# yanielc/medical-vision-textural-bias

Hardware: AMD Instinct MI355X
Metric: BraTS 4ch 240^3 vols/sec filtered+train-step @1/2/4/8 GPU; filter HBM GB/s (higher is better)
Workload: dtype f32

## Files before the change

include/texbias.h:

```cpp
#ifndef TEXBIAS_H
#define TEXBIAS_H

#include <stddef.h>
#include <stdint.h>

#ifdef __cplusplus
extern "C" {
#endif

#define TB_VERSION 1

#define TB_OK 0
#define TB_ERR_INVALID_ARG 1
#define TB_ERR_UNSUPPORTED_SIZE 2
#define TB_ERR_HIP 3
#define TB_ERR_WORKSPACE 4

#define TB_OP_NONE 0
#define TB_OP_DISK 1
#define TB_OP_GIBBS 2
#define TB_OP_LAYER 3
#define TB_OP_WRAP 4
#define TB_OP_SPIKE 5
#define TB_OP_ZF 6
// ... 37 lines not shown

int tb_salt_pepper_f32(const float* x, float* y, int8_t* cls, const float* u_in, uint64_t seed, uint64_t offset,
                       const float* thr, const uint32_t* minmax, int B, int64_t rows, int len, int64_t ld,
                       int64_t sb, void* stream);

int tb_minmax_f32(const float* x, uint32_t* minmax, int B, int64_t rows, int len, int64_t ld, int64_t sb,
                  void* stream);

float tb_key_to_float(uint32_t key);

int tb_disk_mask_f32(float* mask, int64_t outer, int n0, int n1, int n2, int int_r, int64_t r2i, float r2f,
                     int inside_off, void* stream);

int tb_kspace_logabs_sum_f32(const tb_plan* plan, const float* x, const int64_t* xs, void* ws, size_t ws_bytes,
                             int B, int C, const tb_sample_ops* ops, double* out, void* stream);

int tb_conv3d_wgrad_f32(const float* G, const float* X, float* dW, int N, int M, int Cc, int Do, int Ho, int Wo, int Di,
                        int Hi, int Wi, int stride, int pad, void* stream);

int64_t tb_conv3d_wgrad_ws_bytes(int N, int M, int Cc, int Do, int Ho, int Wo, int Di, int Hi, int Wi, int stride,
                                 int pad);
int tb_conv3d_wgrad_ws_f32(const float* G, const float* X, float* dW, int N, int M, int Cc, int Do, int Ho, int Wo,
                           int Di, int Hi, int Wi, int stride, int pad, void* ws, size_t ws_bytes, void* stream);

int tb_conv3d_wgrad_config(int N, int M, int Cc, int Do, int Ho, int Wo, int Di, int Hi, int Wi, int stride, int pad,
                           int64_t* cfg);

int tb_dice_sums_f32(const float* x, const float* t, double* sums, int64_t NC, int64_t S, int sigmoid, int squared,
                     void* stream);
size_t tb_dice_sums_ws_bytes(int64_t NC, int64_t S);
int tb_dice_sums_ws_f32(const float* x, const float* t, double* sums, int64_t NC, int64_t S, int sigmoid, int squared,
                        void* ws, size_t ws_bytes, void* stream);
int tb_dice_metric_sums_f32(const float* x, const float* t, double* sums, int64_t NC, int64_t S, void* stream);
int tb_dice_sums_bwd_f32(const float* x, const float* t, const float* g, float* dx, int64_t NC, int64_t S, int sigmoid,
                         int squared, void* stream);
int tb_dice_loss_f32(const double* sums, float* loss, int64_t NC, int64_t C, int batch, int reduction, float smooth_nr,
                     float smooth_dr, void* stream);
int tb_dice_loss_bwd_f32(const double* sums, const float* gloss, float* gsums, int64_t NC, int64_t C, int batch,
                         int reduction, float smooth_nr, float smooth_dr, void* stream);

int tb_channel_sum_f32(const float* x, float* out, int64_t N, int64_t C, int64_t S, void* stream);
size_t tb_channel_sum_ws_bytes(int64_t N, int64_t C, int64_t S);
int tb_channel_sum_ws_f32(const float* x, float* out, int64_t N, int64_t C, int64_t S, void* ws, size_t ws_bytes,
                          void* stream);

int tb_conv3d_small_f32(const float* x, const float* w, const float* b, float* y, int N, int Cin, int Cout, int D,
// ... 111 lines not shown
```

medical-vision-textural-bias_amd/csrc/conv_wgrad.hip:

```cpp
#include <hip/hip_runtime.h>

#include <cstdlib>

#include "num_cu.h"
#include "texbias.h"

namespace {

typedef float f32x4 __attribute__((ext_vector_type(4)));

constexpr int NT = 256;
constexpr int LDS_FLOATS = 78 * 1024 / 4;
constexpr int kSlack = 16;

struct WgArgs {
  const float* G;
  const float* X;
  float* dW;
  int M, Cc, Do, Ho, Wo, Di, Hi, Wi;
  int YB, YR, Wo4, XP, PG, PC, ncc, ctiles, nyb, xcols;
  int64_t nchunks;
};

typedef __attribute__((address_space(1))) const void* gptr_t;
// ... 390 lines not shown
  }
  __syncthreads();
  if (wave < 2) {
#pragma unroll
    for (int j = 0; j < 27; ++j)
#pragma unroll
      for (int rr = 0; rr < 4; ++rr) red[((j * 2 + wave) * 4 + rr) * 64 + lane] = acc[j][rr];
  }
  __syncthreads();
  float* pt = a.part ? a.part + ((int64_t)blockIdx.y * gridDim.x + blockIdx.x) * (16 * 16 * 27) : nullptr;
  for (int e = tid; e < 27 * 4 * 64; e += NT) {
    const int ln = e & 63, rr = (e >> 6) & 3, j = e >> 8;
    const int m = (ln >> 4) * 4 + rr, c = ln & 15;
    const float v = red[((j * 2 + 0) * 4 + rr) * 64 + ln] + red[((j * 2 + 1) * 4 + rr) * 64 + ln];
    if (pt) {
      pt[(m * 16 + c) * 27 + j] = v;
    } else if (m < mv && c < cv) {
      atomicAdd(&a.dW[((int64_t)(m0 + m) * a.Cc + (c0 + c)) * 27 + j], v);
    }
  }
}

__global__ __launch_bounds__(1024) void k_wgrad_reduce(const float* __restrict__ part, float* __restrict__ dW, int nblk,
                                                       int TM, int TC, int ctiles, int M, int Cc) {
  __shared__ float red[16][64];
  const int tid = (int)threadIdx.x, el = tid & 63, bg = tid >> 6;
  const int TE = TM * TC * 27, tile = (int)blockIdx.y;
  const int e = (int)blockIdx.x * 64 + el;
  const float* src = part + (int64_t)tile * nblk * TE + (e < TE ? e : 0);
  float s0 = 0.f, s1 = 0.f, s2 = 0.f, s3 = 0.f;
  int b = bg;
  for (; b + 48 < nblk; b += 64) {
    s0 += src[(int64_t)b * TE];
    s1 += src[(int64_t)(b + 16) * TE];
    s2 += src[(int64_t)(b + 32) * TE];
    s3 += src[(int64_t)(b + 48) * TE];
  }
  for (; b < nblk; b += 16) s0 += src[(int64_t)b * TE];
  red[bg][el] = (s0 + s1) + (s2 + s3);
  __syncthreads();
  if (bg == 0 && e < TE) {
    float v = 0.f;
#pragma unroll
    for (int g = 0; g < 16; ++g) v += red[g][el];
    const int mt = tile / ctiles, ct = tile - mt * ctiles;
    const int m = e / (TC * 27), r = e - m * (TC * 27), c = r / 27, j = r - c * 27;
    if (mt * TM + m < M && ct * TC + c < Cc) dW[((int64_t)(mt * TM + m) * Cc + ct * TC + c) * 27 + j] = v;
  }
}
// ... 333 lines not shown
    for (int j = 0; j < 9; ++j)
#pragma unroll
      for (int rr = 0; rr < 4; ++rr) red[(((t * 9 + j) * NW + wave) * 4 + rr) * 64 + lane] = acc[t][j][rr];
  __syncthreads();
  float* pt = a.part ? a.part + ((int64_t)blockIdx.y * gridDim.x + blockIdx.x) * (16 * MT * Cc * 27) : nullptr;
  for (int e = tid; e < MT * 9 * 4 * 64; e += NT) {
    const int ln = e & 63, rr = (e >> 6) & 3, tj = e >> 8, t = tj / 9, j = tj - 9 * t;
    const int m = 16 * t + (ln >> 4) * 4 + rr, col = ln & 15;
    if ((!pt && m >= mv) || col >= 3 * Cc) continue;
    float v = 0.f;
#pragma unroll
    for (int w = 0; w < NW; ++w) v += red[((tj * NW + w) * 4 + rr) * 64 + ln];
    const int c = col / 3, tx = col - 3 * c;
    if (pt) pt[(m * Cc + c) * 27 + j * 3 + tx] = v;
    else atomicAdd(&a.dW[((int64_t)(m0 + m) * Cc + c) * 27 + j * 3 + tx], v);
  }
}

struct Zf1Args {
  const float* G;
  const float* X;
  float* dW;
  float* part;
  int N, M, Cc, D, H, W;
  int YB, nyb, ZS, zlen;
  int GR, GM, GS;
  int XR, XC, XS;
};

template <int YB, int WV>
__global__ __launch_bounds__(256) void k_conv3d_wgrad_zf1(Zf1Args a) {
  extern __shared__ __attribute__((aligned(16))) float smem[];
  const int tid = (int)threadIdx.x, lane = tid & 63;
  const int wave = __builtin_amdgcn_readfirstlane(tid >> 6);
  const int W = a.W, H = a.H, D = a.D, M = a.M, Cc = a.Cc;
  float* gsl = smem;
  float* xsl = smem + 4 * a.GS;
  int b = (int)blockIdx.x;
  const int zs = b % a.ZS;
  b /= a.ZS;
  const int yb = b % a.nyb, n = b / a.nyb;
  const int y0 = yb * YB;
  const int z0 = zs * a.zlen, z1 = min(D, z0 + a.zlen);
  for (int i = tid; i < 4 * a.GS + 2 * a.XS; i += 256) smem[i] = 0.f;
  const int64_t plane = (int64_t)H * W, plane4 = plane / 4;
  const float* Gb = a.G + (int64_t)n * M * D * plane;
  const float* Xb = a.X + (int64_t)n * Cc * D * plane;
  const int W4v = W >> 2;
  constexpr int NXL = (5 * YB * WV + 255) / 256, NGL = (3 * (YB + 2) * WV + 255) / 256;
  int xg[NXL], xl[NXL], gg[NGL], gl[NGL];
#pragma unroll
  for (int j = 0; j < NXL; ++j) {
    const int i = tid + 256 * j;
    const int q = i % W4v, t = i / W4v, yy = t % YB, c = t / YB;
    const bool ok = c < Cc && y0 + yy < H;
    xg[j] = ok ? (int)(((int64_t)c * D) * plane4 + ((y0 + yy) * W + 4 * q) / 4) : -1;
    xl[j] = c * a.XC + yy * a.XR + 4 + 4 * q;
  }
#pragma unroll
  for (int j = 0; j < NGL; ++j) {
    const int i = tid + 256 * j;
    const int q = i % W4v, t = i / W4v, r = t % (YB + 2), m = t / (YB + 2);
    const int y = y0 - 1 + r;
    const bool ok = m < M && y >= 0 && y < H;
    gg[j] = ok ? (int)(((int64_t)m * D) * plane4 + (y * W + 4 * q) / 4) : -1;
    gl[j] = m * a.GM + r * a.GR + 4 * q;
  }
  constexpr int ZP = 3;
  float4 rx[ZP][NXL], rg[ZP][NGL];
  auto load_x = [&](int zi, float4 (&r)[NXL]) {
    const float4* src = reinterpret_cast<const float4*>(Xb) + (int64_t)(zi < D ? zi : D - 1) * plane4;
#pragma unroll
    for (int j = 0; j < NXL; ++j) {
      const float4 v = src[xg[j] < 0 ? 0 : xg[j]];
      r[j] = xg[j] < 0 ? make_float4(0.f, 0.f, 0.f, 0.f) : v;
    }
  };
  auto store_x = [&](int slot, const float4 (&r)[NXL]) {
#pragma unroll
    for (int j = 0; j < NXL; ++j)
      if (xg[j] >= 0) *reinterpret_cast<float4*>(xsl + slot * a.XS + xl[j]) = r[j];
  };
  auto load_g = [&](int pz, float4 (&r)[NGL]) {
    const bool in = pz >= 0 && pz < D;
    const float4* src = reinterpret_cast<const float4*>(Gb) + (int64_t)(in ? pz : 0) * plane4;
#pragma unroll
    for (int j = 0; j < NGL; ++j) {
      const float4 v = src[gg[j] < 0 ? 0 : gg[j]];
      r[j] = (in && gg[j] >= 0) ? v : make_float4(0.f, 0.f, 0.f, 0.f);
    }
  };
  auto store_g = [&](int slot, const float4 (&r)[NGL], int) {
#pragma unroll
    for (int j = 0; j < NGL; ++j)
      if (gg[j] >= 0) *reinterpret_cast<float4*>(gsl + slot * a.GS + gl[j]) = r[j];
  };
  __syncthreads();
  load_g(z0 - 1, rg[0]);
  store_g((z0 + 3) & 3, rg[0], z0 - 1);
  load_g(z0, rg[0]);
  store_g(z0 & 3, rg[0], z0);
#pragma unroll
  for (int p = 0; p < ZP; ++p) {
    load_x(z0 + p, rx[p]);
    load_g(z0 + p + 1, rg[p]);
  }
  const int li = lane & 15, lk = lane >> 4;
  int atz[2], aoff[2];
  bool aok[2];
#pragma unroll
  for (int t = 0; t < 2; ++t) {
    const int r = 16 * t + li, m = r / 9, tz = (r / 3) % 3, ty = r % 3;
    aok[t] = m < M;
    atz[t] = tz;
    aoff[t] = aok[t] ? m * a.GM + (2 - ty) * a.GR + lk : 0;
  }
  const int bc = li / 3, btx = li - 3 * bc;
  const bool bok = bc < Cc;
  const int boff = bok ? bc * a.XC + 3 + btx + lk : 0;
  const int kpr = W >> 2, np = 4 / YB, yy = wave % YB, part = wave / YB;
  const int kb = (kpr * part) / np, ke = (kpr * (part + 1)) / np;
  f32x4 acc[2][2];
#pragma unroll
  for (int t = 0; t < 2; ++t) acc[0][t] = acc[1][t] = f32x4{0.f, 0.f, 0.f, 0.f};
  auto step = [&](int zi, float4 (&rxp)[NXL], float4 (&rgp)[NGL]) {
    store_x(zi & 1, rxp);
    store_g((zi + 1) & 3, rgp, zi + 1);
    __syncthreads();
    if (zi + ZP < z1) {
      load_x(zi + ZP, rxp);
      load_g(zi + ZP + 1, rgp);
    }
    const float* ga0 = gsl + ((zi + 1 - atz[0]) & 3) * a.GS + aoff[0] + yy * a.GR;
    const float* ga1 = gsl + ((zi + 1 - atz[1]) & 3) * a.GS + aoff[1] + yy * a.GR;
    const float* xb = xsl + (zi & 1) * a.XS + boff + yy * a.XR;
    auto ld = [&](int k, float& v0, float& v1, float& u) {
      const int px = 4 * (k < ke ? k : ke - 1);
      v0 = aok[0] ? ga0[px] : 0.f;
      v1 = aok[1] ? ga1[px] : 0.f;
      u = bok ? xb[px] : 0.f;
    };
    if (kb < ke) {
      float p0, p1, pu, q0, q1, qu;
      ld(kb, p0, p1, pu);
      int k = kb;
      for (; k + 1 < ke; k += 2) {
        ld(k + 1, q0, q1, qu);
        acc[0][0] = __builtin_amdgcn_mfma_f32_16x16x4f32(p0, pu, acc[0][0], 0, 0, 0);
        acc[0][1] = __builtin_amdgcn_mfma_f32_16x16x4f32(p1, pu, acc[0][1], 0, 0, 0);
        ld(k + 2, p0, p1, pu);
        acc[1][0] = __builtin_amdgcn_mfma_f32_16x16x4f32(q0, qu, acc[1][0], 0, 0, 0);
        acc[1][1] = __builtin_amdgcn_mfma_f32_16x16x4f32(q1, qu, acc[1][1], 0, 0, 0);
      }
      if (k < ke) {
        acc[0][0] = __builtin_amdgcn_mfma_f32_16x16x4f32(p0, pu, acc[0][0], 0, 0, 0);
        acc[0][1] = __builtin_amdgcn_mfma_f32_16x16x4f32(p1, pu, acc[0][1], 0, 0, 0);
      }
    }
  };
  for (int zi = z0; zi < z1; zi += ZP) {
    step(zi, rx[0], rg[0]);
    if (zi + 1 < z1) step(zi + 1, rx[1], rg[1]);
    if (zi + 2 < z1) step(zi + 2, rx[2], rg[2]);
  }
  __syncthreads();
  float* red = smem;
#pragma unroll
  for (int t = 0; t < 2; ++t)
#pragma unroll
    for (int rr = 0; rr < 4; ++rr) red[((t * 4 + wave) * 4 + rr) * 64 + lane] = acc[0][t][rr] + acc[1][t][rr];
  __syncthreads();
  float* pt = a.part ? a.part + (int64_t)blockIdx.x * (M * Cc * 27) : nullptr;
  for (int e = tid; e < 2 * 4 * 64; e += 256) {
    const int ln = e & 63, rr = (e >> 6) & 3, t = e >> 8;
    const int r = 16 * t + 4 * (ln >> 4) + rr, col = ln & 15;
    const int m = r / 9, c = col / 3;
    if (m >= M || c >= Cc) continue;
    const int tz = (r / 3) % 3, ty = r % 3, tx = col - 3 * c;
    const float v = red[((t * 4 + 0) * 4 + rr) * 64 + ln] + red[((t * 4 + 1) * 4 + rr) * 64 + ln] +
                    red[((t * 4 + 2) * 4 + rr) * 64 + ln] + red[((t * 4 + 3) * 4 + rr) * 64 + ln];
    if (pt) pt[(m * Cc + c) * 27 + tz * 9 + ty * 3 + tx] = v;
    else atomicAdd(&a.dW[((int64_t)m * Cc + c) * 27 + tz * 9 + ty * 3 + tx], v);
  }
}

int pad_mod32(int v, int rem) {
  while ((v & 31) != rem) ++v;
  return v;
}

template <int S, int TX, int SEG>
int launch(const WgArgs& a, int blocks_y, size_t lds, hipStream_t st) {
  static const hipError_t attr = hipFuncSetAttribute(reinterpret_cast<const void*>(&k_conv3d_wgrad<S, TX, SEG>),
                                                     hipFuncAttributeMaxDynamicSharedMemorySize, 163840);
  if (attr != hipSuccess) return TB_ERR_HIP;
  constexpr int target = 512;
  int64_t gx = (target + blocks_y - 1) / blocks_y;
  if (gx > a.nchunks) gx = a.nchunks;
  if (gx < 1) gx = 1;
  hipLaunchKernelGGL((k_conv3d_wgrad<S, TX, SEG>), dim3((unsigned)gx, (unsigned)blocks_y), dim3(NT), lds, st, a);
  return hipGetLastError() == hipSuccess ? TB_OK : TB_ERR_HIP;
}

template <int S, int TX>
int launch_seg(const WgArgs& a, int seg, int by, size_t lds, hipStream_t st) {
  switch (seg) {
// ... 251 lines not shown
template <int YB, int MT>
int launch_zf2_t(const Zf2Args& a, size_t lds, dim3 grid, hipStream_t st) {
  auto kern = a.Wo <= 40 ? k_conv3d_wgrad_zf2<YB, MT, 10, 8> : k_conv3d_wgrad_zf2<YB, MT, 20, 8>;
  const hipError_t attr = hipFuncSetAttribute(reinterpret_cast<const void*>(kern),
                                              hipFuncAttributeMaxDynamicSharedMemorySize, 163840);
  if (attr != hipSuccess) return TB_ERR_HIP;
  hipLaunchKernelGGL(kern, grid, dim3(512), lds, st, a);
  return hipGetLastError() == hipSuccess ? TB_OK : TB_ERR_HIP;
}
int launch_zf2(const Zf2Args& a, int MT, size_t lds, dim3 grid, hipStream_t st) {
  if (MT == 1) return a.YB == 4 ? launch_zf2_t<4, 1>(a, lds, grid, st) : a.YB == 2 ? launch_zf2_t<2, 1>(a, lds, grid, st) : launch_zf2_t<1, 1>(a, lds, grid, st);
  return a.YB == 4 ? launch_zf2_t<4, 2>(a, lds, grid, st) : a.YB == 2 ? launch_zf2_t<2, 2>(a, lds, grid, st) : launch_zf2_t<1, 2>(a, lds, grid, st);
}

bool use_zf1(int M, int Cc, int stride, int Do, int Ho, int Wo, int Di, int Hi, int Wi, const void* G, const void* X) {
  constexpr bool on = true;
  return on && stride == 1 && M <= 3 && Cc <= 5 && Do == Di && Ho == Hi && Wo == Wi && Wo % 4 == 0 && Wo <= 256 &&
         (reinterpret_cast<uintptr_t>(G) & 15) == 0 && (reinterpret_cast<uintptr_t>(X) & 15) == 0;
}

int zf1_setup(Zf1Args& a, size_t& lds, dim3& grid, int N, int M, int Cc, int D, int H, int W, int ncu) {
  a.N = N; a.M = M; a.Cc = Cc; a.D = D; a.H = H; a.W = W;
  constexpr int yb_env = 0;
  a.GR = pad_mod32(W, 4);
  a.XR = pad_mod32(W + 8, 4);
  a.YB = 0;
  for (int yb : {2, 4, 1}) {
    if (yb_env && yb != yb_env) continue;
    const int gm = pad_mod32((yb + 2) * a.GR, 12), gs = pad_mod32(M * gm, 20);
    const int xc = pad_mod32(yb * a.XR, 8), xs = pad_mod32(Cc * xc, 16);
    const size_t bytes = (size_t)4 * (4 * gs + 2 * xs);
    if (bytes <= 81920) {
      a.YB = yb; a.GM = gm; a.GS = gs; a.XC = xc; a.XS = xs;
      lds = bytes > (size_t)2 * 4 * 4 * 64 * 4 ? bytes : (size_t)2 * 4 * 4 * 64 * 4;
      break;
    }
  }
  if (!a.YB) return TB_ERR_UNSUPPORTED_SIZE;
  a.nyb = (H + a.YB - 1) / a.YB;
  const int base = N * a.nyb;
  int best = 1 << 30;
  a.zlen = D;
  for (int zl = D; zl >= 1; --zl) {
    const int zs = (D + zl - 1) / zl;
    const int rounds = (base * zs + 2 * ncu - 1) / (2 * ncu);
    const int cost = rounds * (zl + 2);
    if (cost < best) {
      best = cost;
      a.zlen = zl;
    }
  }
  a.ZS = (D + a.zlen - 1) / a.zlen;
  grid = dim3((unsigned)(N * a.nyb * a.ZS));
  return TB_OK;
}

template <int YB>
// ... 98 lines not shown
  if (pad != 1 || N < 1) return r;
  const int ncu = tb::num_cu();
  if (use_zm(M, Cc, stride, Do, Ho, Wo, Di, Hi, Wi, G, X) &&
      zm_setup(r.zm, r.lds, r.grid, N, M, Cc, Do, Ho, Wo, ncu) == TB_OK) {
    r.kind = 1, r.TM = 16, r.TC = 16, r.ctiles = r.zm.ctiles;
  } else if (use_zm2(M, Cc, stride, Do, Ho, Wo, Di, Hi, Wi, G, X) &&
             zm2_setup(r.zm2, r.lds, r.grid, N, M, Cc, Do, Ho, Wo, Di, Hi, Wi, ncu) == TB_OK) {
    r.kind = 2, r.TM = 32, r.TC = 16, r.ctiles = r.zm2.ctiles;
  } else if (use_zf1(M, Cc, stride, Do, Ho, Wo, Di, Hi, Wi, G, X) &&
             zf1_setup(r.zf1, r.lds, r.grid, N, M, Cc, Do, Ho, Wo, ncu) == TB_OK) {
    r.kind = 3, r.TM = M, r.TC = Cc, r.ctiles = 1;
  } else if (use_zf2(M, Cc, stride, Do, Ho, Wo, Di, Hi, Wi, G, X) &&
             zf2_setup(r.zf2, r.MT, r.lds, r.grid, N, M, Cc, Do, Ho, Wo, Di, Hi, Wi, ncu) == TB_OK) {
    r.kind = 4, r.TM = 16 * r.MT, r.TC = Cc, r.ctiles = 1;
  }
  return r;
}

int64_t tb_conv3d_wgrad_ws_bytes(int N, int M, int Cc, int Do, int Ho, int Wo, int Di, int Hi, int Wi, int stride,
                                 int pad) {
  return (int64_t)zroute(N, M, Cc, Do, Ho, Wo, Di, Hi, Wi, stride, pad, nullptr, nullptr).bytes();
}

int tb_conv3d_wgrad_ws_f32(const float* G, const float* X, float* dW, int N, int M, int Cc, int Do, int Ho, int Wo,
                           int Di, int Hi, int Wi, int stride, int pad, void* ws, size_t ws_bytes, void* stream) {
  if (!G || !X || !dW) return TB_ERR_INVALID_ARG;
  hipStream_t st = reinterpret_cast<hipStream_t>(stream);
  ZRoute r = zroute(N, M, Cc, Do, Ho, Wo, Di, Hi, Wi, stride, pad, G, X);
  if (!ws || !r.kind || ws_bytes < r.bytes() || (reinterpret_cast<uintptr_t>(ws) & 3) != 0)
    return tb_conv3d_wgrad_f32(G, X, dW, N, M, Cc, Do, Ho, Wo, Di, Hi, Wi, stride, pad, stream);
  float* part = static_cast<float*>(ws);
  int rc = TB_OK;
  switch (r.kind) {
    case 1: r.zm.G = G, r.zm.X = X, r.zm.dW = dW, r.zm.part = part; rc = launch_zm(r.zm, r.lds, r.grid, st); break;
    case 2: r.zm2.G = G, r.zm2.X = X, r.zm2.dW = dW, r.zm2.part = part; rc = launch_zm2(r.zm2, r.lds, r.grid, st); break;
    case 3: r.zf1.G = G, r.zf1.X = X, r.zf1.dW = dW, r.zf1.part = part; rc = launch_zf1(r.zf1, r.lds, r.grid, st); break;
    default: r.zf2.G = G, r.zf2.X = X, r.zf2.dW = dW, r.zf2.part = part; rc = launch_zf2(r.zf2, r.MT, r.lds, r.grid, st); break;
  }
  if (rc != TB_OK) return rc;
  hipLaunchKernelGGL(k_wgrad_reduce, dim3((r.TM * r.TC * 27 + 63) / 64, r.grid.y), dim3(1024), 0, st,
                     static_cast<const float*>(part), dW, (int)r.grid.x, r.TM, r.TC, r.ctiles, M, Cc);
  return hipGetLastError() == hipSuccess ? TB_OK : TB_ERR_HIP;
}

int tb_conv3d_wgrad_config(int N, int M, int Cc, int Do, int Ho, int Wo, int Di, int Hi, int Wi, int stride, int pad,
                           int64_t* cfg) {
  if (!cfg) return TB_ERR_INVALID_ARG;
  WgArgs a{};
  int seg = 0, TX = 0, by = 0;
  size_t lds = 0;
  const int rc = wg_setup(a, seg, TX, by, lds, N, M, Cc, Do, Ho, Wo, Di, Hi, Wi, stride, pad);
  if (rc != TB_OK) return rc;
  cfg[0] = seg; cfg[1] = TX; cfg[2] = a.YB; cfg[3] = a.nchunks; cfg[4] = (int64_t)lds;
  return TB_OK;
}
```

medical-vision-textural-bias_amd/texbias/_lib.py:

```python
from __future__ import annotations

import ctypes as C
import os
import threading

from ._abi import TB_OK

PKG_DIR = os.path.dirname(os.path.dirname(os.path.abspath(__file__)))
LIB_PATH = os.environ.get("TEXBIAS_LIB", os.path.join(PKG_DIR, "libtexbias.so"))

_lock = threading.Lock()
_lib = None


class TexbiasError(RuntimeError):
    pass


def _proto(L):
    P, I, I64, U64, F, SZ = C.c_void_p, C.c_int, C.c_int64, C.c_uint64, C.c_float, C.c_size_t
    sig = {
        "tb_version": (I, []),
        "tb_error_string": (C.c_char_p, [I]),
        "tb_last_hip_error": (I, []),
        "tb_plan_create": (I, [I, I, I, C.POINTER(P)]),
        "tb_plan_destroy": (I, [P]),
        "tb_workspace_bytes": (SZ, [P, I]),
        "tb_plan_radices": (I, [P, I, P]),
        "tb_kspace_filter_f32": (I, [P, P, P, P, P, I, P, SZ, I, I, P, P, P]),
        "tb_planes_closed_form_f32": (I, [P, P, P, P, P, I, P, SZ, I, I, P, P, P]),
        "tb_salt_pepper_f32": (I, [P, P, P, P, U64, U64, P, P, I, I64, I, I64, I64, P]),
        "tb_minmax_f32": (I, [P, P, I, I64, I, I64, I64, P]),
        "tb_key_to_float": (F, [C.c_uint32]),
        "tb_disk_mask_f32": (I, [P, I64, I, I, I, I, I64, F, I, P]),
        "tb_kspace_logabs_sum_f32": (I, [P, P, P, P, SZ, I, I, P, P, P]),
        "tb_conv3d_wgrad_f32": (I, [P, P, P] + [I] * 11 + [P]),
        "tb_conv3d_wgrad_config": (I, [I] * 11 + [P]),
        "tb_conv3d_wgrad_ws_bytes": (I64, [I] * 11),
        "tb_conv3d_wgrad_ws_f32": (I, [P, P, P] + [I] * 11 + [P, SZ, P]),
        "tb_instnorm_prelu_workspace_bytes": (SZ, [I64]),
        "tb_instnorm_prelu_fwd_f32": (I, [P, P, P, P, P, I64, I64, F, P, SZ, P]),
        "tb_instnorm_prelu_bwd_f32": (I, [P, P, P, P, P, P, P, I64, I64, P, SZ, P]),
        "tb_channel_sum_f32": (I, [P, P, I64, I64, I64, P]),
        "tb_channel_sum_ws_bytes": (SZ, [I64, I64, I64]),
        "tb_channel_sum_ws_f32": (I, [P, P, I64, I64, I64, P, SZ, P]),
        "tb_adn_workspace_bytes": (SZ, [I64, I64, I64]),
        "tb_adam_f32": (I, [I, P, P, P, P, P, P, P] + [C.c_double] * 5 + [I, P]),
        "tb_adn_counters": (I64, [I64, I64]),
        "tb_adn_fwd_f32": (I, [P, I64, P, I64, P, I64, P, P, P, I64, I64, I64, F, P, SZ, P, P]),
        "tb_adn_bwd_f32": (I, [P, I64, P, I64, P, I64, P, P, P, P, P, P, I64, I64, I64, P, SZ, P, P]),
        "tb_conv3d_small_f32": (I, [P, P, P, P] + [I] * 6 + [P]),
        "tb_conv3d_small_add_f32": (I, [P, P, P, P, P] + [I] * 6 + [P]),
        "tb_conv3d_fwd16_add_f32": (I, [P, P, P, P, P] + [I] * 4 + [P]),
        "tb_conv3d_mfma_add_f32": (I, [P, P, P, P, P] + [I] * 5 + [P]),
        "tb_conv3d_mfma_dgrad_f32": (I, [P, P, P, I64, P] + [I] * 5 + [P]),
        "tb_conv3d_fwd16_dgrad_f32": (I, [P, P, P, I64, P] + [I] * 4 + [P]),
        "tb_conv3d_s2_fewin_f32": (I, [P, P, P, P] + [I] * 6 + [P]),
        "tb_convT3d_fewout_f32": (I, [P, P, P, P] + [I] * 6 + [P]),
        "tb_conv3d_fwd16_f32": (I, [P, P, P, P] + [I] * 4 + [P]),
        "tb_convT3d_mfma64_f32": (I, [P, P, P, P] + [I] * 4 + [P]),
        "tb_convT3d_mfma_f32": (I, [P, P, P, P] + [I] * 5 + [P]),
        "tb_conv3d_mfma_f32": (I, [P, P, P, P] + [I] * 5 + [P]),
# ... 60 lines not shown
```

medical-vision-textural-bias_amd/texbias/conv.py:

```python
from __future__ import annotations

import functools
import math
import os

import torch
import torch.nn as nn
import torch.nn.functional as F

from ._lib import TexbiasError, check, lib

MIN_K_PER_OUTPUT = 64
ENABLED = os.environ.get("TEXBIAS_WGRAD", "1") != "0"
CONVT64 = True
CONVMFMA = True
CONV16 = True


def _stream(t: torch.Tensor) -> int:
    return torch.cuda.current_stream(t.device).cuda_stream


@functools.lru_cache(maxsize=256)
def _wgrad_ws_bytes(N, M, Cc, Do, Ho, Wo, Di, Hi, Wi, stride, pad) -> int:
    return int(lib().tb_conv3d_wgrad_ws_bytes(N, M, Cc, Do, Ho, Wo, Di, Hi, Wi, stride, pad))


def wgrad(G: torch.Tensor, X: torch.Tensor, w_shape, stride: int, pad: int) -> torch.Tensor:
    G = G.contiguous()
    X = X.contiguous()
    N, M = G.shape[:2]
    Cc = X.shape[1]
    dW = torch.empty((M, Cc, 3, 3, 3), dtype=torch.float32, device=G.device)
    Do, Ho, Wo = G.shape[2:]
    Di, Hi, Wi = X.shape[2:]
    nb = _wgrad_ws_bytes(N, M, Cc, Do, Ho, Wo, Di, Hi, Wi, stride, pad)
    ws = torch.empty(max(nb, 4), dtype=torch.uint8, device=G.device) if nb > 0 else None
    with torch.cuda.device(G.device):
        check(lib().tb_conv3d_wgrad_ws_f32(G.data_ptr(), X.data_ptr(), dW.data_ptr(), N, M, Cc, Do, Ho, Wo, Di, Hi, Wi,
                                           stride, pad, ws.data_ptr() if ws is not None else None, nb,
                                           _stream(G)), "tb_conv3d_wgrad_ws_f32")
    return dW.view(w_shape)


def wgrad_config(g_shape, x_shape, stride: int, pad: int = 1) -> dict:
    import ctypes
    cfg = (ctypes.c_int64 * 5)()
    N, M, Do, Ho, Wo = g_shape
    Cc, Di, Hi, Wi = x_shape[1:]
    check(lib().tb_conv3d_wgrad_config(N, M, Cc, Do, Ho, Wo, Di, Hi, Wi, stride, pad, cfg), "tb_conv3d_wgrad_config")
    return dict(zip(("SEG", "TX", "YB", "chunks", "lds_bytes"), list(cfg)))


def channel_sum(g: torch.Tensor) -> torch.Tensor:
    g = g.contiguous()
    N, Cc = g.shape[:2]
    S = g[0, 0].numel()
    out = torch.empty(Cc, dtype=torch.float32, device=g.device)
    nb = int(lib().tb_channel_sum_ws_bytes(N, Cc, S))
    ws = torch.empty(nb, dtype=torch.uint8, device=g.device)
    with torch.cuda.device(g.device):
        check(lib().tb_channel_sum_ws_f32(g.data_ptr(), out.data_ptr(), N, Cc, S, ws.data_ptr(), nb, _stream(g)),
              "tb_channel_sum_ws_f32")
    return out

# ... 477 lines not shown
            return small_conv(gy, w.flip(2, 3, 4).transpose(0, 1).contiguous(), None)
        if k == "fewout":
            return conv_s2_fewin(gy, s2_pairs(w), None, w.shape[0])
        if k == "convT64":
            return convT_mfma(gy if gy.data_ptr() % 16 == 0 else gy.clone(), w, None)
        if k == "gemm":
            return gemm_dgrad(gy, w, self.stride[0], self.transposed)
        gx, _, _ = torch.ops.aten.convolution_backward(
            gy, x, w, None, list(self.stride), list(self.padding), [1, 1, 1], self.transposed,
            list(self.output_padding), 1, [True, False, False])
        return gx

    def weight_grad(self, gy, x, w):
        if self.wgg:
            G, X = (x, gy) if self.transposed else (gy, x)
            return wgrad_gemm(G, X, w.shape, self.stride[0], self.k)
        if self.fast_w and tuple(w.shape[2:]) == (3, 3, 3) and self.padding[0] == 1:
            return weight_grad(gy, x, w, self.stride[0], self.transposed, self.output_padding)
        _, gw, _ = torch.ops.aten.convolution_backward(
            gy, x, w, None, list(self.stride), list(self.padding), [1, 1, 1], self.transposed,
            list(self.output_padding), 1, [False, True, False])
        return gw

    def backward(self, gy, x, w, need_x: bool, need_w: bool, need_b: bool, gb=None):
        gy = gy.contiguous()
        gx = self.input_grad(gy, x, w) if need_x else None
        gw = self.weight_grad(gy, x, w) if need_w else None
        if need_b and gb is None:
            gb = channel_sum(gy) if self.kind != "aten" else gy.sum(dim=(0, 2, 3, 4))
        return gx, gw, gb if need_b else None


class _RouteFn(torch.autograd.Function):
    @staticmethod
    def forward(ctx, x, w, b, route):
        y = route.forward(x.contiguous() if route.kind != "aten" else x, w, b)
        ctx.save_for_backward(x, w)
        ctx.route, ctx.has_b = route, b is not None
        return y

    @staticmethod
    def backward(ctx, gy):
        x, w = ctx.saved_tensors
        n = ctx.needs_input_grad
        gx, gw, gb = ctx.route.backward(gy, x, w, n[0], n[1], n[2] and ctx.has_b)
        return gx, gw, gb, None


def route_of(mod, x: torch.Tensor) -> "Route":
    key = (tuple(x.shape), x.dtype, x.device, x.data_ptr() % 16 == 0, x.is_contiguous())
# ... 24 lines not shown
```

medical-vision-textural-bias_amd/texbias/unet.py:

```python
from __future__ import annotations

import os
from typing import Sequence

import torch
import torch.nn as nn

from . import conv as _conv
from .conv import Conv3d, ConvTranspose3d
from . import norm as _norm
from .norm import adn_backward, adn_forward, instnorm_prelu

FUSED = os.environ.get("TEXBIAS_FUSED_UNITS", "1") != "0"


def _fusable(x: torch.Tensor, conv: nn.Module, adn) -> bool:
    if not (FUSED and _norm.ENABLED and x.is_cuda and x.dtype == torch.float32 and
            isinstance(conv, (Conv3d, ConvTranspose3d)) and conv.groups == 1 and conv.dilation == (1, 1, 1) and
            _conv.custom_backward_applies(x, conv.weight)):
        return False
    if isinstance(conv, Conv3d) and conv.padding_mode != "zeros":
        return False
    return adn is None or adn.D.p == 0.0 or not adn.training

# ... 18 lines not shown
        if ctx.res_is_x:
            gx = ctx.route.input_grad(dz, x, w, add=g) if n[0] else None
            return gx, gw, db, da, None, None, None, None, None
        gx = ctx.route.input_grad(dz, x, w) if n[0] else None
        return gx, gw, db, da, None, None, (g if ctx.has_res and n[6] else None), None, None


class _ConvResFn(torch.autograd.Function):

    @staticmethod
    def forward(ctx, x, w, b, route):
        x = x.contiguous()
        y = route.forward(x, w, b, add=x)
        ctx.save_for_backward(x, w)
        ctx.route, ctx.has_b = route, b is not None
        return y

    @staticmethod
    def backward(ctx, g):
        x, w = ctx.saved_tensors
        n = ctx.needs_input_grad
        g = g.contiguous()
        gx = ctx.route.input_grad(g, x, w, add=g) if n[0] else None
        gw = ctx.route.weight_grad(g, x, w) if n[1] else None
        gb = _conv.channel_sum(g) if ctx.has_b and n[2] else None
        return gx, gw, gb, None


def _adjacent(a: torch.Tensor, b: torch.Tensor):
    if not (a.is_contiguous() and b.is_contiguous() and a.shape[1:] == b.shape[1:] and a.dtype == b.dtype and
            a.untyped_storage().data_ptr() == b.untyped_storage().data_ptr() and
            b.storage_offset() == a.storage_offset() + a.numel()):
        return None
    return torch.empty(0, dtype=a.dtype, device=a.device).set_(
        a.untyped_storage(), a.storage_offset(), (a.shape[0] + b.shape[0],) + tuple(a.shape[1:]))


class _StackedUnitFn(torch.autograd.Function):

    @staticmethod
    def forward(ctx, x, w0, b0, wr, br, a0w, w1, b1, a1w, unit, eps, skip):
        c = w0.shape[0]
        w_st = _adjacent(w0, wr)
        if w_st is None:
            w_st = torch.cat([w0, wr], 0)
        b_st = None
        if b0 is not None and br is not None:
            b_st = _adjacent(b0, br)
# ... 263 lines not shown
```

Before: 166.8.

## Fuse bias gradient into zf1 weight-gradient kernel and vectorize its LDS inner loop

Result: faster. 170.2, median of 6 (+2.0%).

```diff
diff --git a/include/texbias.h b/include/texbias.h
--- a/include/texbias.h
+++ b/include/texbias.h
@@ -83,6 +83,12 @@
                                  int pad);
 int tb_conv3d_wgrad_ws_f32(const float* G, const float* X, float* dW, int N, int M, int Cc, int Do, int Ho, int Wo,
                            int Di, int Hi, int Wi, int stride, int pad, void* ws, size_t ws_bytes, void* stream);
+
+int64_t tb_conv3d_wgrad_bias_ws_bytes(int N, int M, int Cc, int Do, int Ho, int Wo, int Di, int Hi, int Wi, int stride,
+                                      int pad, int* sums_bias);
+int tb_conv3d_wgrad_bias_ws_f32(const float* G, const float* X, float* dW, float* dbias, int N, int M, int Cc, int Do,
+                                int Ho, int Wo, int Di, int Hi, int Wi, int stride, int pad, void* ws, size_t ws_bytes,
+                                int* bias_done, void* stream);
 
 int tb_conv3d_wgrad_config(int N, int M, int Cc, int Do, int Ho, int Wo, int Di, int Hi, int Wi, int stride, int pad,
                            int64_t* cfg);
diff --git a/medical-vision-textural-bias_amd/csrc/conv_wgrad.hip b/medical-vision-textural-bias_amd/csrc/conv_wgrad.hip
--- a/medical-vision-textural-bias_amd/csrc/conv_wgrad.hip
+++ b/medical-vision-textural-bias_amd/csrc/conv_wgrad.hip
@@ -436,9 +436,26 @@
 }
 
 __global__ __launch_bounds__(1024) void k_wgrad_reduce(const float* __restrict__ part, float* __restrict__ dW, int nblk,
-                                                       int TM, int TC, int ctiles, int M, int Cc) {
+                                                       int TM, int TC, int ctiles, int M, int Cc,
+                                                       const double* __restrict__ bpart, float* __restrict__ dbias) {
   __shared__ float red[16][64];
+  __shared__ double bred[1024];
   const int tid = (int)threadIdx.x, el = tid & 63, bg = tid >> 6;
+  if (bpart && blockIdx.x == gridDim.x - 1) {
+    for (int m = 0; m < M; ++m) {
+      double s = 0.0;
+      for (int b = tid; b < nblk; b += 1024) s += bpart[(int64_t)b * M + m];
+      bred[tid] = s;
+      __syncthreads();
+      for (int w = 512; w; w >>= 1) {
+        if (tid < w) bred[tid] += bred[tid + w];
+        __syncthreads();
+      }
+      if (tid == 0) dbias[m] = (float)bred[0];
+      __syncthreads();
+    }
+    return;
+  }
   const int TE = TM * TC * 27, tile = (int)blockIdx.y;
   const int e = (int)blockIdx.x * 64 + el;
   const float* src = part + (int64_t)tile * nblk * TE + (e < TE ? e : 0);
@@ -818,11 +835,14 @@
   const float* X;
   float* dW;
   float* part;
+  double* bpart;
   int N, M, Cc, D, H, W;
   int YB, nyb, ZS, zlen;
   int GR, GM, GS;
   int XR, XC, XS;
 };
+
+constexpr size_t ZF1_RED_BYTES = (size_t)2 * 4 * 4 * 64 * 4;
 
 template <int YB, int WV>
 __global__ __launch_bounds__(256) void k_conv3d_wgrad_zf1(Zf1Args a) {
@@ -832,6 +852,8 @@
   const int W = a.W, H = a.H, D = a.D, M = a.M, Cc = a.Cc;
   float* gsl = smem;
   float* xsl = smem + 4 * a.GS;
+  f32x4* smem4 = reinterpret_cast<f32x4*>(smem);
+  const int dump = a.GS + (a.XS >> 1) + tid;
   int b = (int)blockIdx.x;
   const int zs = b % a.ZS;
   b /= a.ZS;
@@ -845,13 +867,14 @@
   const int W4v = W >> 2;
   constexpr int NXL = (5 * YB * WV + 255) / 256, NGL = (3 * (YB + 2) * WV + 255) / 256;
   int xg[NXL], xl[NXL], gg[NGL], gl[NGL];
+  bool own[NGL];
 #pragma unroll
   for (int j = 0; j < NXL; ++j) {
     const int i = tid + 256 * j;
     const int q = i % W4v, t = i / W4v, yy = t % YB, c = t / YB;
     const bool ok = c < Cc && y0 + yy < H;
     xg[j] = ok ? (int)(((int64_t)c * D) * plane4 + ((y0 + yy) * W + 4 * q) / 4) : -1;
-    xl[j] = c * a.XC + yy * a.XR + 4 + 4 * q;
+    xl[j] = ok ? a.GS + ((c * a.XC + yy * a.XR) >> 2) + 1 + q : dump;
   }
 #pragma unroll
   for (int j = 0; j < NGL; ++j) {
@@ -860,104 +883,123 @@
     const int y = y0 - 1 + r;
     const bool ok = m < M && y >= 0 && y < H;
     gg[j] = ok ? (int)(((int64_t)m * D) * plane4 + (y * W + 4 * q) / 4) : -1;
-    gl[j] = m * a.GM + r * a.GR + 4 * q;
+    gl[j] = ok ? ((m * a.GM + r * a.GR) >> 2) + q : dump;
+    own[j] = ok && r >= 1 && r <= YB;
   }
   constexpr int ZP = 3;
-  float4 rx[ZP][NXL], rg[ZP][NGL];
-  auto load_x = [&](int zi, float4 (&r)[NXL]) {
-    const float4* src = reinterpret_cast<const float4*>(Xb) + (int64_t)(zi < D ? zi : D - 1) * plane4;
-#pragma unroll
-    for (int j = 0; j < NXL; ++j) {
-      const float4 v = src[xg[j] < 0 ? 0 : xg[j]];
-      r[j] = xg[j] < 0 ? make_float4(0.f, 0.f, 0.f, 0.f) : v;
-    }
-  };
-  auto store_x = [&](int slot, const float4 (&r)[NXL]) {
+  f32x4 rx0[NXL], rx1[NXL], rx2[NXL], rg0[NGL], rg1[NGL], rg2[NGL];
+  double bs[NGL];
+#pragma unroll
+  for (int j = 0; j < NGL; ++j) bs[j] = 0.0;
+  const bool bias = a.bpart != nullptr;
+  auto load_x = [&](int zi, f32x4 (&r)[NXL]) {
+    const f32x4* src = reinterpret_cast<const f32x4*>(Xb) + (int64_t)(zi < D ? zi : D - 1) * plane4;
+#pragma unroll
+    for (int j = 0; j < NXL; ++j) r[j] = src[xg[j] < 0 ? 0 : xg[j]];
+  };
+  auto store_x = [&](int slot, const f32x4 (&r)[NXL]) {
 #pragma unroll
     for (int j = 0; j < NXL; ++j)
-      if (xg[j] >= 0) *reinterpret_cast<float4*>(xsl + slot * a.XS + xl[j]) = r[j];
-  };
-  auto load_g = [&](int pz, float4 (&r)[NGL]) {
+      smem4[(xg[j] >= 0 ? slot * (a.XS >> 2) : 0) + xl[j]] = r[j];
+  };
+  auto load_g = [&](int pz, f32x4 (&r)[NGL]) {
+    const f32x4* src = reinterpret_cast<const f32x4*>(Gb) + (int64_t)(pz >= 0 && pz < D ? pz : 0) * plane4;
+#pragma unroll
+    for (int j = 0; j < NGL; ++j) r[j] = src[gg[j] < 0 ? 0 : gg[j]];
+  };
+  auto store_g = [&](int slot, const f32x4 (&r)[NGL], int pz) {
     const bool in = pz >= 0 && pz < D;
-    const float4* src = reinterpret_cast<const float4*>(Gb) + (int64_t)(in ? pz : 0) * plane4;
+    const bool cnt = bias && pz >= z0 && pz < z1;
 #pragma unroll
     for (int j = 0; j < NGL; ++j) {
-      const float4 v = src[gg[j] < 0 ? 0 : gg[j]];
-      r[j] = (in && gg[j] >= 0) ? v : make_float4(0.f, 0.f, 0.f, 0.f);
-    }
-  };
-  auto store_g = [&](int slot, const float4 (&r)[NGL], int) {
-#pragma unroll
-    for (int j = 0; j < NGL; ++j)
-      if (gg[j] >= 0) *reinterpret_cast<float4*>(gsl + slot * a.GS + gl[j]) = r[j];
+      const f32x4 v = in ? r[j] : f32x4{0.f, 0.f, 0.f, 0.f};
+      smem4[(gg[j] >= 0 ? slot * (a.GS >> 2) : 0) + gl[j]] = v;
+      const float q = (v[0] + v[1]) + (v[2] + v[3]);
+      bs[j] += (double)(own[j] && cnt ? q : 0.f);
+    }
   };
   __syncthreads();
-  load_g(z0 - 1, rg[0]);
-  store_g((z0 + 3) & 3, rg[0], z0 - 1);
-  load_g(z0, rg[0]);
-  store_g(z0 & 3, rg[0], z0);
-#pragma unroll
-  for (int p = 0; p < ZP; ++p) {
-    load_x(z0 + p, rx[p]);
-    load_g(z0 + p + 1, rg[p]);
-  }
+  load_g(z0 - 1, rg0);
+  store_g((z0 + 3) & 3, rg0, z0 - 1);
+  load_g(z0, rg0);
+  store_g(z0 & 3, rg0, z0);
+  load_x(z0, rx0);
+  load_g(z0 + 1, rg0);
+  load_x(z0 + 1, rx1);
+  load_g(z0 + 2, rg1);
+  load_x(z0 + 2, rx2);
+  load_g(z0 + 3, rg2);
   const int li = lane & 15, lk = lane >> 4;
   int atz[2], aoff[2];
-  bool aok[2];
 #pragma unroll
   for (int t = 0; t < 2; ++t) {
-    const int r = 16 * t + li, m = r / 9, tz = (r / 3) % 3, ty = r % 3;
-    aok[t] = m < M;
+    const int r0 = 16 * t + li, r = r0 < 9 * M ? r0 : 0;
+    const int m = r / 9, tz = (r / 3) % 3, ty = r % 3;
     atz[t] = tz;
-    aoff[t] = aok[t] ? m * a.GM + (2 - ty) * a.GR + lk : 0;
-  }
-  const int bc = li / 3, btx = li - 3 * bc;
-  const bool bok = bc < Cc;
-  const int boff = bok ? bc * a.XC + 3 + btx + lk : 0;
-  const int kpr = W >> 2, np = 4 / YB, yy = wave % YB, part = wave / YB;
-  const int kb = (kpr * part) / np, ke = (kpr * (part + 1)) / np;
+    aoff[t] = m * a.GM + (2 - ty) * a.GR + 4 * lk;
+  }
+  const int col = li < 3 * Cc ? li : 0, bc = col / 3, btx = col - 3 * bc;
+  const int boff = bc * a.XC + 3 + btx + 4 * lk;
+  const int ngr = (W + 15) >> 4, np = 4 / YB, yy = wave % YB, part = wave / YB;
+  const int gb = (ngr * part) / np, ge = (ngr * (part + 1)) / np;
   f32x4 acc[2][2];
 #pragma unroll
   for (int t = 0; t < 2; ++t) acc[0][t] = acc[1][t] = f32x4{0.f, 0.f, 0.f, 0.f};
-  auto step = [&](int zi, float4 (&rxp)[NXL], float4 (&rgp)[NGL]) {
+  auto mm = [&](const f32x4& v0, const f32x4& v1, const f32x4& u) {
+#pragma unroll
+    for (int s = 0; s < 4; ++s) {
+      acc[s & 1][0] = __builtin_amdgcn_mfma_f32_16x16x4f32(v0[s], u[s], acc[s & 1][0], 0, 0, 0);
+      acc[s & 1][1] = __builtin_amdgcn_mfma_f32_16x16x4f32(v1[s], u[s], acc[s & 1][1], 0, 0, 0);
+    }
+  };
+  auto step = [&](int zi, f32x4 (&rxp)[NXL], f32x4 (&rgp)[NGL]) {
     store_x(zi & 1, rxp);
     store_g((zi + 1) & 3, rgp, zi + 1);
     __syncthreads();
-    if (zi + ZP < z1) {
-      load_x(zi + ZP, rxp);
-      load_g(zi + ZP + 1, rgp);
-    }
-    const float* ga0 = gsl + ((zi + 1 - atz[0]) & 3) * a.GS + aoff[0] + yy * a.GR;
-    const float* ga1 = gsl + ((zi + 1 - atz[1]) & 3) * a.GS + aoff[1] + yy * a.GR;
+    load_x(zi + ZP, rxp);
+    load_g(zi + ZP + 1, rgp);
+    const f32x4* ga0 = reinterpret_cast<const f32x4*>(gsl + ((zi + 1 - atz[0]) & 3) * a.GS + aoff[0] + yy * a.GR);
+    const f32x4* ga1 = reinterpret_cast<const f32x4*>(gsl + ((zi + 1 - atz[1]) & 3) * a.GS + aoff[1] + yy * a.GR);
     const float* xb = xsl + (zi & 1) * a.XS + boff + yy * a.XR;
-    auto ld = [&](int k, float& v0, float& v1, float& u) {
-      const int px = 4 * (k < ke ? k : ke - 1);
-      v0 = aok[0] ? ga0[px] : 0.f;
-      v1 = aok[1] ? ga1[px] : 0.f;
-      u = bok ? xb[px] : 0.f;
+    auto ld = [&](int g, f32x4& v0, f32x4& v1, f32x4& u) {
+      v0 = ga0[4 * g];
+      v1 = ga1[4 * g];
+      const float* p = xb + 16 * g;
+      u = f32x4{p[0], p[1], p[2], p[3]};
     };
-    if (kb < ke) {
-      float p0, p1, pu, q0, q1, qu;
-      ld(kb, p0, p1, pu);
-      int k = kb;
-      for (; k + 1 < ke; k += 2) {
-        ld(k + 1, q0, q1, qu);
-        acc[0][0] = __builtin_amdgcn_mfma_f32_16x16x4f32(p0, pu, acc[0][0], 0, 0, 0);
-        acc[0][1] = __builtin_amdgcn_mfma_f32_16x16x4f32(p1, pu, acc[0][1], 0, 0, 0);
-        ld(k + 2, p0, p1, pu);
-        acc[1][0] = __builtin_amdgcn_mfma_f32_16x16x4f32(q0, qu, acc[1][0], 0, 0, 0);
-        acc[1][1] = __builtin_amdgcn_mfma_f32_16x16x4f32(q1, qu, acc[1][1], 0, 0, 0);
-      }
-      if (k < ke) {
-        acc[0][0] = __builtin_amdgcn_mfma_f32_16x16x4f32(p0, pu, acc[0][0], 0, 0, 0);
-        acc[0][1] = __builtin_amdgcn_mfma_f32_16x16x4f32(p1, pu, acc[0][1], 0, 0, 0);
-      }
-    }
-  };
-  for (int zi = z0; zi < z1; zi += ZP) {
-    step(zi, rx[0], rg[0]);
-    if (zi + 1 < z1) step(zi + 1, rx[1], rg[1]);
-    if (zi + 2 < z1) step(zi + 2, rx[2], rg[2]);
+    if (gb < ge) {
+      f32x4 p0, p1, pu, q0, q1, qu;
+      ld(gb, p0, p1, pu);
+      int g = gb;
+      for (; g + 2 < ge; g += 2) {
+        ld(g + 1, q0, q1, qu);
+        __builtin_amdgcn_sched_barrier(0);
+        mm(p0, p1, pu);
+        __builtin_amdgcn_sched_barrier(0);
+        ld(g + 2, p0, p1, pu);
+        __builtin_amdgcn_sched_barrier(0);
+        mm(q0, q1, qu);
+        __builtin_amdgcn_sched_barrier(0);
+      }
+      if (g + 1 < ge) {
+        ld(g + 1, q0, q1, qu);
+        __builtin_amdgcn_sched_barrier(0);
+        mm(p0, p1, pu);
+        mm(q0, q1, qu);
+      } else {
+        mm(p0, p1, pu);
+      }
+    }
+  };
+  int zi = z0;
+  for (; zi + ZP <= z1; zi += ZP) {
+    step(zi, rx0, rg0);
+    step(zi + 1, rx1, rg1);
+    step(zi + 2, rx2, rg2);
+  }
+  if (zi < z1) {
+    step(zi, rx0, rg0);
+    if (zi + 1 < z1) step(zi + 1, rx1, rg1);
   }
   __syncthreads();
   float* red = smem;
@@ -965,7 +1007,21 @@
   for (int t = 0; t < 2; ++t)
 #pragma unroll
     for (int rr = 0; rr < 4; ++rr) red[((t * 4 + wave) * 4 + rr) * 64 + lane] = acc[0][t][rr] + acc[1][t][rr];
+  double* bred = reinterpret_cast<double*>(reinterpret_cast<char*>(smem) + ZF1_RED_BYTES);
+  if (bias) {
+#pragma unroll
+    for (int mm_ = 0; mm_ < 3; ++mm_) {
+      double v = 0.0;
+#pragma unroll
+      for (int j = 0; j < NGL; ++j) v += ((tid + 256 * j) / W4v) / (YB + 2) == mm_ ? bs[j] : 0.0;
+#pragma unroll
+      for (int off = 32; off; off >>= 1) v += __shfl_down(v, off);
+      if (lane == 0) bred[wave * 3 + mm_] = v;
+    }
+  }
   __syncthreads();
+  if (bias && tid < M)
+    a.bpart[(int64_t)blockIdx.x * M + tid] = (bred[tid] + bred[3 + tid]) + (bred[6 + tid] + bred[9 + tid]);
   float* pt = a.part ? a.part + (int64_t)blockIdx.x * (M * Cc * 27) : nullptr;
   for (int e = tid; e < 2 * 4 * 64; e += 256) {
     const int ln = e & 63, rr = (e >> 6) & 3, t = e >> 8;
@@ -978,6 +1034,11 @@
     if (pt) pt[(m * Cc + c) * 27 + tz * 9 + ty * 3 + tx] = v;
     else atomicAdd(&a.dW[((int64_t)m * Cc + c) * 27 + tz * 9 + ty * 3 + tx], v);
   }
+}
+
+int pad_mod(int v, int mod, int rem) {
+  while (v % mod != rem) ++v;
+  return v;
 }
 
 int pad_mod32(int v, int rem) {
@@ -1275,17 +1336,19 @@
 int zf1_setup(Zf1Args& a, size_t& lds, dim3& grid, int N, int M, int Cc, int D, int H, int W, int ncu) {
   a.N = N; a.M = M; a.Cc = Cc; a.D = D; a.H = H; a.W = W;
   constexpr int yb_env = 0;
-  a.GR = pad_mod32(W, 4);
-  a.XR = pad_mod32(W + 8, 4);
+  const int Wp = (W + 15) & ~15;
+  a.GR = pad_mod(Wp, 64, 40);
+  a.XR = pad_mod32(Wp + 8, 4);
   a.YB = 0;
   for (int yb : {2, 4, 1}) {
     if (yb_env && yb != yb_env) continue;
-    const int gm = pad_mod32((yb + 2) * a.GR, 12), gs = pad_mod32(M * gm, 20);
+    const int gm = pad_mod((yb + 2) * a.GR, 64, 24), gs = pad_mod(M * gm, 64, 56);
     const int xc = pad_mod32(yb * a.XR, 8), xs = pad_mod32(Cc * xc, 16);
-    const size_t bytes = (size_t)4 * (4 * gs + 2 * xs);
+    const size_t bytes = (size_t)4 * (4 * gs + 2 * xs + 4 * 256);
     if (bytes <= 81920) {
       a.YB = yb; a.GM = gm; a.GS = gs; a.XC = xc; a.XS = xs;
-      lds = bytes > (size_t)2 * 4 * 4 * 64 * 4 ? bytes : (size_t)2 * 4 * 4 * 64 * 4;
+      const size_t red = ZF1_RED_BYTES + 4 * 3 * sizeof(double);
+      lds = bytes > red ? bytes : red;
       break;
     }
   }
@@ -1430,25 +1493,54 @@
   return (int64_t)zroute(N, M, Cc, Do, Ho, Wo, Di, Hi, Wi, stride, pad, nullptr, nullptr).bytes();
 }
 
-int tb_conv3d_wgrad_ws_f32(const float* G, const float* X, float* dW, int N, int M, int Cc, int Do, int Ho, int Wo,
-                           int Di, int Hi, int Wi, int stride, int pad, void* ws, size_t ws_bytes, void* stream) {
+static size_t bias_off(const ZRoute& r) { return (r.bytes() + 7) & ~(size_t)7; }
+static size_t bias_bytes(const ZRoute& r, int M) { return r.kind == 3 ? (size_t)r.grid.x * M * sizeof(double) : 0; }
+
+int64_t tb_conv3d_wgrad_bias_ws_bytes(int N, int M, int Cc, int Do, int Ho, int Wo, int Di, int Hi, int Wi, int stride,
+                                      int pad, int* sums_bias) {
+  const ZRoute r = zroute(N, M, Cc, Do, Ho, Wo, Di, Hi, Wi, stride, pad, nullptr, nullptr);
+  const size_t bb = bias_bytes(r, M);
+  if (sums_bias) *sums_bias = bb ? 1 : 0;
+  return (int64_t)(bb ? bias_off(r) + bb : r.bytes());
+}
+
+int tb_conv3d_wgrad_bias_ws_f32(const float* G, const float* X, float* dW, float* dbias, int N, int M, int Cc, int Do,
+                                int Ho, int Wo, int Di, int Hi, int Wi, int stride, int pad, void* ws, size_t ws_bytes,
+                                int* bias_done, void* stream) {
+  if (bias_done) *bias_done = 0;
   if (!G || !X || !dW) return TB_ERR_INVALID_ARG;
   hipStream_t st = reinterpret_cast<hipStream_t>(stream);
   ZRoute r = zroute(N, M, Cc, Do, Ho, Wo, Di, Hi, Wi, stride, pad, G, X);
   if (!ws || !r.kind || ws_bytes < r.bytes() || (reinterpret_cast<uintptr_t>(ws) & 3) != 0)
     return tb_conv3d_wgrad_f32(G, X, dW, N, M, Cc, Do, Ho, Wo, Di, Hi, Wi, stride, pad, stream);
   float* part = static_cast<float*>(ws);
+  double* bpart = nullptr;
+  if (dbias && bias_bytes(r, M) && ws_bytes >= bias_off(r) + bias_bytes(r, M) &&
+      (reinterpret_cast<uintptr_t>(ws) & 7) == 0)
+    bpart = reinterpret_cast<double*>(static_cast<char*>(ws) + bias_off(r));
   int rc = TB_OK;
   switch (r.kind) {
     case 1: r.zm.G = G, r.zm.X = X, r.zm.dW = dW, r.zm.part = part; rc = launch_zm(r.zm, r.lds, r.grid, st); break;
     case 2: r.zm2.G = G, r.zm2.X = X, r.zm2.dW = dW, r.zm2.part = part; rc = launch_zm2(r.zm2, r.lds, r.grid, st); break;
-    case 3: r.zf1.G = G, r.zf1.X = X, r.zf1.dW = dW, r.zf1.part = part; rc = launch_zf1(r.zf1, r.lds, r.grid, st); break;
+    case 3:
+      r.zf1.G = G, r.zf1.X = X, r.zf1.dW = dW, r.zf1.part = part, r.zf1.bpart = bpart;
+      rc = launch_zf1(r.zf1, r.lds, r.grid, st);
+      break;
     default: r.zf2.G = G, r.zf2.X = X, r.zf2.dW = dW, r.zf2.part = part; rc = launch_zf2(r.zf2, r.MT, r.lds, r.grid, st); break;
   }
   if (rc != TB_OK) return rc;
-  hipLaunchKernelGGL(k_wgrad_reduce, dim3((r.TM * r.TC * 27 + 63) / 64, r.grid.y), dim3(1024), 0, st,
-                     static_cast<const float*>(part), dW, (int)r.grid.x, r.TM, r.TC, r.ctiles, M, Cc);
-  return hipGetLastError() == hipSuccess ? TB_OK : TB_ERR_HIP;
+  hipLaunchKernelGGL(k_wgrad_reduce, dim3((r.TM * r.TC * 27 + 63) / 64 + (bpart ? 1 : 0), r.grid.y), dim3(1024), 0, st,
+                     static_cast<const float*>(part), dW, (int)r.grid.x, r.TM, r.TC, r.ctiles, M, Cc,
+                     static_cast<const double*>(bpart), dbias);
+  if (hipGetLastError() != hipSuccess) return TB_ERR_HIP;
+  if (bias_done) *bias_done = bpart ? 1 : 0;
+  return TB_OK;
+}
+
+int tb_conv3d_wgrad_ws_f32(const float* G, const float* X, float* dW, int N, int M, int Cc, int Do, int Ho, int Wo,
+                           int Di, int Hi, int Wi, int stride, int pad, void* ws, size_t ws_bytes, void* stream) {
+  return tb_conv3d_wgrad_bias_ws_f32(G, X, dW, nullptr, N, M, Cc, Do, Ho, Wo, Di, Hi, Wi, stride, pad, ws, ws_bytes,
+                                     nullptr, stream);
 }
 
 int tb_conv3d_wgrad_config(int N, int M, int Cc, int Do, int Ho, int Wo, int Di, int Hi, int Wi, int stride, int pad,
diff --git a/medical-vision-textural-bias_amd/texbias/_lib.py b/medical-vision-textural-bias_amd/texbias/_lib.py
--- a/medical-vision-textural-bias_amd/texbias/_lib.py
+++ b/medical-vision-textural-bias_amd/texbias/_lib.py
@@ -38,6 +38,8 @@
         "tb_conv3d_wgrad_config": (I, [I] * 11 + [P]),
         "tb_conv3d_wgrad_ws_bytes": (I64, [I] * 11),
         "tb_conv3d_wgrad_ws_f32": (I, [P, P, P] + [I] * 11 + [P, SZ, P]),
+        "tb_conv3d_wgrad_bias_ws_bytes": (I64, [I] * 11 + [P]),
+        "tb_conv3d_wgrad_bias_ws_f32": (I, [P, P, P, P] + [I] * 11 + [P, SZ, P, P]),
         "tb_instnorm_prelu_workspace_bytes": (SZ, [I64]),
         "tb_instnorm_prelu_fwd_f32": (I, [P, P, P, P, P, I64, I64, F, P, SZ, P]),
         "tb_instnorm_prelu_bwd_f32": (I, [P, P, P, P, P, P, P, I64, I64, P, SZ, P]),
diff --git a/medical-vision-textural-bias_amd/texbias/conv.py b/medical-vision-textural-bias_amd/texbias/conv.py
--- a/medical-vision-textural-bias_amd/texbias/conv.py
+++ b/medical-vision-textural-bias_amd/texbias/conv.py
@@ -41,6 +41,36 @@
                                            stride, pad, ws.data_ptr() if ws is not None else None, nb,
                                            _stream(G)), "tb_conv3d_wgrad_ws_f32")
     return dW.view(w_shape)
+
+
+@functools.lru_cache(maxsize=256)
+def _wgrad_bias_ws_bytes(N, M, Cc, Do, Ho, Wo, Di, Hi, Wi, stride, pad):
+    import ctypes
+    sums = ctypes.c_int(0)
+    nb = int(lib().tb_conv3d_wgrad_bias_ws_bytes(N, M, Cc, Do, Ho, Wo, Di, Hi, Wi, stride, pad, ctypes.byref(sums)))
+    return nb, bool(sums.value)
+
+
+def wgrad_bias(G: torch.Tensor, X: torch.Tensor, w_shape, stride: int, pad: int):
+    import ctypes
+    G = G.contiguous()
+    X = X.contiguous()
+    N, M = G.shape[:2]
+    Cc = X.shape[1]
+    Do, Ho, Wo = G.shape[2:]
+    Di, Hi, Wi = X.shape[2:]
+    nb, sums = _wgrad_bias_ws_bytes(N, M, Cc, Do, Ho, Wo, Di, Hi, Wi, stride, pad)
+    if not sums:
+        return wgrad(G, X, w_shape, stride, pad), None
+    dW = torch.empty((M, Cc, 3, 3, 3), dtype=torch.float32, device=G.device)
+    gb = torch.empty(M, dtype=torch.float32, device=G.device)
+    ws = torch.empty(max(nb, 8), dtype=torch.uint8, device=G.device)
+    done = ctypes.c_int(0)
+    with torch.cuda.device(G.device):
+        check(lib().tb_conv3d_wgrad_bias_ws_f32(G.data_ptr(), X.data_ptr(), dW.data_ptr(), gb.data_ptr(), N, M, Cc, Do, Ho,
+                                                Wo, Di, Hi, Wi, stride, pad, ws.data_ptr(), nb, ctypes.byref(done),
+                                                _stream(G)), "tb_conv3d_wgrad_bias_ws_f32")
+    return dW.view(w_shape), (gb if done.value else None)
 
 
 def wgrad_config(g_shape, x_shape, stride: int, pad: int = 1) -> dict:
@@ -564,10 +594,19 @@
             list(self.output_padding), 1, [False, True, False])
         return gw
 
+    def weight_bias_grad(self, gy, x, w):
+        if not self.wgg and not self.transposed and self.fast_w and tuple(w.shape[2:]) == (3, 3, 3) and \
+                self.padding[0] == 1 and _wgrad_tiles(tuple(gy.shape), tuple(x.shape), self.stride[0]):
+            return wgrad_bias(gy, x, w.shape, self.stride[0], 1)
+        return self.weight_grad(gy, x, w), None
+
     def backward(self, gy, x, w, need_x: bool, need_w: bool, need_b: bool, gb=None):
         gy = gy.contiguous()
         gx = self.input_grad(gy, x, w) if need_x else None
-        gw = self.weight_grad(gy, x, w) if need_w else None
+        if need_w and need_b and gb is None:
+            gw, gb = self.weight_bias_grad(gy, x, w)
+        else:
+            gw = self.weight_grad(gy, x, w) if need_w else None
         if need_b and gb is None:
             gb = channel_sum(gy) if self.kind != "aten" else gy.sum(dim=(0, 2, 3, 4))
         return gx, gw, gb if need_b else None
diff --git a/medical-vision-textural-bias_amd/texbias/unet.py b/medical-vision-textural-bias_amd/texbias/unet.py
--- a/medical-vision-textural-bias_amd/texbias/unet.py
+++ b/medical-vision-textural-bias_amd/texbias/unet.py
@@ -64,8 +64,14 @@
         n = ctx.needs_input_grad
         g = g.contiguous()
         gx = ctx.route.input_grad(g, x, w, add=g) if n[0] else None
-        gw = ctx.route.weight_grad(g, x, w) if n[1] else None
-        gb = _conv.channel_sum(g) if ctx.has_b and n[2] else None
+        need_b = ctx.has_b and n[2]
+        gb = None
+        if n[1] and need_b:
+            gw, gb = ctx.route.weight_bias_grad(g, x, w)
+        else:
+            gw = ctx.route.weight_grad(g, x, w) if n[1] else None
+        if need_b and gb is None:
+            gb = _conv.channel_sum(g)
         return gx, gw, gb, None
 
 
```
